# FlowEternal/multitask-hydranet

Hardware: AMD Instinct MI355X
Metric: images/sec (fwd+bwd) HydraNet @ default res, 1/2/4/8 MI355X; CPU-ref same run (higher is better)
Workload: dtype bf16

## Files before the change

### multitask_hydranet_amd/csrc/hn_gemm.hip

```cpp
#include "hn_common.h"
#include <climits>

#ifdef HN_TUNING
#define HN_DBG(p) ((p).dbg)
#else
#define HN_DBG(p) 0
#endif

struct XSrc {
    const bf16* x0;
    const bf16* x1;
    int mode;
    int H, W;
    int Hi, Wi;
    int C0, C1;
    int ld0, ld1;
    int up;
    long M;
    int clamp;
    int diag;
};

__device__ __forceinline__ int border_idx(int v, int L, int clamp) {
    if (clamp == 2) return (v < 0 || v >= L) ? -1 : v;
// ... 20 lines not shown
        iy = iy < 0 ? -iy : (iy >= s.Hi ? 2 * s.Hi - 2 - iy : iy);
        ix = ix < 0 ? -ix : (ix >= s.Wi ? 2 * s.Wi - 2 - ix : ix);
        if (c < s.C0) {
            const int hh = s.Hi >> s.up, ww = s.Wi >> s.up;
            return ld8(s.x0 + (((long)n * hh + (iy >> s.up)) * ww + (ix >> s.up)) * s.ld0 + c);
        }
        return ld8(s.x1 + (((long)n * s.Hi + iy) * s.Wi + ix) * s.ld1 + (c - s.C0));
    }
    const int iy = oy - ky, ix = ox - kx;
    if (iy < 0 || iy >= s.Hi || ix < 0 || ix >= s.Wi) return zero8();
    return ld8(s.x0 + (((long)n * s.Hi + iy) * s.Wi + ix) * s.ld0 + c);
}

__device__ __attribute__((aligned(16))) bf16 g_zero_piece[8];

__device__ __forceinline__ const bf16* x_piece_ptr(const XSrc& s, long m, int n, int oy, int ox, int tap, int c) {
    if (m >= s.M || c >= s.C0 + s.C1) return g_zero_piece;
    if (s.mode == 0) return s.x0 + m * s.ld0 + c;
    if (s.mode == 1) return s.x0 + (((long)n * s.Hi + 2 * oy) * s.Wi + 2 * ox) * s.ld0 + c;
    const int ky = (tap * 11) >> 5, kx = tap - 3 * ky;
    if (s.mode == 2) {
        int iy = oy + ky - 1, ix = ox + kx - 1;
        iy = iy < 0 ? -iy : (iy >= s.Hi ? 2 * s.Hi - 2 - iy : iy);
        ix = ix < 0 ? -ix : (ix >= s.Wi ? 2 * s.Wi - 2 - ix : ix);
        if (c < s.C0) {
            const int hh = s.Hi >> s.up, ww = s.Wi >> s.up;
            return s.x0 + (((long)n * hh + (iy >> s.up)) * ww + (ix >> s.up)) * s.ld0 + c;
        }
        return s.x1 + (((long)n * s.Hi + iy) * s.Wi + ix) * s.ld1 + (c - s.C0);
    }
    const int iy = oy - ky, ix = ox - kx;
    if (iy < 0 || iy >= s.Hi || ix < 0 || ix >= s.Wi) return g_zero_piece;
    return s.x0 + (((long)n * s.Hi + iy) * s.Wi + ix) * s.ld0 + c;
}

__device__ __forceinline__ long pixel_off(const XSrc& s, long m, int n, int oy, int ox, int tap, int which) {
    if (m >= s.M) return -1;
    if (s.mode == 0) return which ? -1 : m * s.ld0;
    if (s.mode == 1) return which ? -1 : (((long)n * s.Hi + 2 * oy) * s.Wi + 2 * ox) * s.ld0;
    const int ky = (tap * 11) >> 5, kx = tap - 3 * ky;
    if (s.mode == 2) {
        int iy = oy + ky - 1, ix = ox + kx - 1;
        iy = iy < 0 ? -iy : (iy >= s.Hi ? 2 * s.Hi - 2 - iy : iy);
        ix = ix < 0 ? -ix : (ix >= s.Wi ? 2 * s.Wi - 2 - ix : ix);
        if (which) return s.C1 ? (((long)n * s.Hi + iy) * s.Wi + ix) * s.ld1 : -1;
        const int hh = s.Hi >> s.up, ww = s.Wi >> s.up;
        return (((long)n * hh + (iy >> s.up)) * ww + (ix >> s.up)) * s.ld0;
    }
    const int iy = oy - ky, ix = ox - kx;
    if (which || iy < 0 || iy >= s.Hi || ix < 0 || ix >= s.Wi) return -1;
    return (((long)n * s.Hi + iy) * s.Wi + ix) * s.ld0;
}

__device__ __forceinline__ void glds16(const bf16* src, char* lds_wave_base) {
    __builtin_amdgcn_global_load_lds((const __attribute__((address_space(1))) void*)src,
                                     (__attribute__((address_space(3))) void*)lds_wave_base, 16, 0, 0);
}

__device__ __forceinline__ int swz(int row, int piece) { return row * 128 + ((piece ^ (row & 7)) << 4); }
__device__ __forceinline__ int pswz32(int row) { return (row >> 1) & 2; }

struct GemmNT {
    XSrc x;
    const bf16* w;
    int Nout, KP, taps;
    const float* bias;
    int act;
    void* out;
    int ldc;
    float* psum;
    float* psq;
    long rpi;
    long img_stride;
    int d2s;
    const float* xscale; const float* xshift; const float* xgate; long xhw; int xact;
    const bf16* addend; int ld_add;
    int phase_mode, phase_span;
    int add_s2;
    long* amax;
    int add_pre;
    long w_img_stride; unsigned w_rpi;
    const float* lcoef; int ln; long lrow[HN_MAX_LEVELS + 1];
    int lo_n; unsigned lo_hw[HN_MAX_LEVELS]; unsigned lo_pix[HN_MAX_LEVELS];
    int fold;
    bf16* fold_out2; int ld_fo2;
    bf16* ring;
    const bf16* fold_y; int ld_fy;
    int emode; const bf16* ez; int ld_ez; const float* ecoef;
    const bf16* ey; int ld_ey;
    int tile_major;
    int wpre;
    unsigned long long* dbg_buf;
    int dbg;
};

struct StatCoef { f32x4 sc, sh, mu, rs; };
__device__ __forceinline__ StatCoef stat_coef(const float* ecoef, int Nout, int emode, int co0, bool ev) {
    StatCoef c;
    c.sc = c.sh = c.mu = c.rs = (f32x4){0.f, 0.f, 0.f, 0.f};
    if (ev) {
        c.sc = *reinterpret_cast<const f32x4*>(ecoef + co0);
        c.sh = *reinterpret_cast<const f32x4*>(ecoef + Nout + co0);
        if (emode == 2) {
            c.mu = *reinterpret_cast<const f32x4*>(ecoef + 2 * Nout + co0);
            c.rs = *reinterpret_cast<const f32x4*>(ecoef + 3 * Nout + co0);
        }
    }
    return c;
}
__device__ __forceinline__ void stat_terms4(int emode, const f32x4 q, const f32x4 z, const StatCoef& cf, float& a0, float& a1, float& a2, float& a3,
                                            float& b0, float& b1, float& b2, float& b3) {
    float t1[4], t2[4];
#pragma unroll
    for (int r = 0; r < 4; ++r) {
        const float pre = cf.sc[r] * z[r] + cf.sh[r];
        const float b = bfround(pre > 0.f ? pre : 0.f);
        const float g = pre > 0.f ? q[r] : 0.f;
        t1[r] = emode == 0 ? q[r] : (emode == 1 ? q[r] * b : g);
        t2[r] = emode == 0 ? q[r] * q[r] : g * (z[r] - cf.mu[r]) * cf.rs[r];
    }
    a0 += t1[0]; a1 += t1[1]; a2 += t1[2]; a3 += t1[3];
    b0 += t2[0]; b1 += t2[1]; b2 += t2[2]; b3 += t2[3];
}

template <int BC, int BP, int WGC, int WGP, bool OUT_F32, int R, bool XF = false, int KG = 1, bool PLAIN = false, bool EPRE = false>
__global__ __launch_bounds__(256 * KG) void gemm_nt_kernel(const GemmNT p) {
    static_assert(!XF || R == 2, "the register-staged operand transform is written for the double buffer");
    static_assert(!PLAIN || !XF, "the plain-rows form has no operand transform");
    static_assert(KG == 1 || (!XF && R == 2), "the K-group form is written for the plain double buffer");
    constexpr int WC = BC / WGC, WP = BP / WGP, TC = WC / 16, TP = WP / 16;
    constexpr int XR = BP / 32, WR = (BC + 31) / 32;
    constexpr int STAGE = (BC + BP) * 128;
    extern __shared__ __attribute__((aligned(16))) char smem[];
    const int tid = threadIdx.x & 255, kg = __builtin_amdgcn_readfirstlane(threadIdx.x >> 8), lane = tid & 63, wave = __builtin_amdgcn_readfirstlane(tid >> 6);
    const int wc = wave / WGP, wp = wave % WGP;
    const int ncy = (p.Nout + BC - 1) / BC;
    const int lid = xcd_remap(blockIdx.x, gridDim.x);
    const int c_tile = lid % ncy, p_tile = lid / ncy;
    const int c_blk = c_tile * BC;
    const long p_blk = (long)p_tile * BP;
    const int r0 = tid >> 3, lp = (tid & 7) ^ (r0 & 7), half = lp >> 2, sub = (lp & 3) * 8;
    const int kc = p.KP >> 5, Q = p.taps * kc, S = (((Q + 1) >> 1) + KG - 1) / KG;
    const int Ktot = p.taps * p.KP;

    int xn[XR], xy[XR], xx[XR];
#pragma unroll
    for (int i = 0; i < XR; ++i) {
        if constexpr (PLAIN) { xn[i] = 0; xy[i] = 0; xx[i] = 0; }
        else decomp_row(p.x, p_blk + r0 + 32 * i, xn[i], xy[i], xx[i]);
    }

    int* ty0 = reinterpret_cast<int*>(smem + R * KG * STAGE);
    int* tx0 = ty0 + 3 * p.x.H;
    int* ty1 = tx0 + 3 * p.x.W;
    int* tx1 = ty1 + 3 * p.x.H;
    if (!PLAIN && p.x.mode >= 2) {
        for (int i = tid; i < 3 * p.x.H; i += 256) {
            const int k = i / p.x.H, o = i - k * p.x.H;
            if (p.x.mode == 2) {
                int v = o + k - 1;
                v = border_idx(v, p.x.Hi, p.x.clamp);
                ty0[i] = v >> p.x.up;
                if (p.x.C1) ty1[i] = v;
            } else {
                const int v = o - k;
                ty0[i] = (v < 0 || v >= p.x.Hi) ? -1 : v;
            }
// ... 427 lines not shown
#pragma unroll
        for (int k = 0; k < WGP; ++k) { t1 += red[(k * BC + tid) * 2]; t2 += red[(k * BC + tid) * 2 + 1]; }
        p.psum[(long)p_tile * p.Nout + c_blk + tid] = t1;
        if (p.psq) p.psq[(long)p_tile * p.Nout + c_blk + tid] = t2;
    }
    if (staged) {
        bf16* outp = reinterpret_cast<bf16*>(p.out);
        float e1[8], e2[8], emu[8], ers[8];
#pragma unroll
        for (int k = 0; k < 8; ++k) { e1[k] = 0.f; e2[k] = 0.f; emu[k] = 0.f; ers[k] = 0.f; }
        if (e3) {
            const int co = c_blk + (tid % NPC) * 8;
            if (co < p.Nout) {
#pragma unroll
                for (int k = 0; k < 8; ++k) { emu[k] = p.ecoef[2 * p.Nout + co + k]; ers[k] = p.ecoef[3 * p.Nout + co + k]; }
            }
        }
#pragma unroll
        for (int u = 0; u < NIT; ++u) {
            const int idx = tid + 256 * u;
            if (idx >= BP * NPC) break;
            const int row = idx / NPC, pc = idx % NPC;
            const long pix = p_blk + row;
            const int co = c_blk + pc * 8;
            if (pix < p.x.M && co < p.Nout) {
                bf16x8 v = *reinterpret_cast<const bf16x8*>(smem + row * (BC * 2) + (((pc ^ row) & (NPC - 1)) << 4));
                long orow = pix * p.ldc;
                if (p.rpi) {
                    const unsigned im = (unsigned)pix / (unsigned)p.rpi;
                    orow = (long)im * p.img_stride + (long)((unsigned)pix - im * (unsigned)p.rpi) * p.ldc;
                }
                if (p.addend && !p.add_pre) {
                    bool has = true;
                    bf16x8 a;
                    if (PRE) {
                        has = phas[u < PRE ? u : 0];
                        a = padd[u < PRE ? u : 0];
                    } else {
                        long arow = pix;
                        if (p.add_s2) {
                            const unsigned W = (unsigned)p.x.W, H = (unsigned)p.x.H;
                            const unsigned x = (unsigned)pix % W, t = (unsigned)pix / W;
                            const unsigned y = t % H, n = t / H;
                            has = !((x | y) & 1u);
                            arow = ((long)n * (H >> 1) + (y >> 1)) * (W >> 1) + (x >> 1);
                        }
                        a = has ? ld8(p.addend + arow * p.ld_add + co) : zero8();
                    }
                    if (has) {
#pragma unroll
                        for (int k = 0; k < 8; ++k) v[k] = f2bf(bf2f(v[k]) + bf2f(a[k]));
                    }
                }
                if (e3) {
                    const bf16x8 yv = PRE ? pey[u < PRE ? u : 0] : ld8(p.ey + pix * p.ld_ey + co);
                    const bf16x8 zv = PRE ? pzz[u < PRE ? u : 0] : ld8(p.ez + pix * p.ld_ez + co);
#pragma unroll
                    for (int k = 0; k < 8; ++k) {
                        const float g = bf2f(yv[k]) > 0.f ? bf2f(v[k]) : 0.f;
                        e1[k] += g;
                        e2[k] += g * (bf2f(zv[k]) - emu[k]) * ers[k];
                    }
                }
                *reinterpret_cast<bf16x8*>(outp + orow + co) = v;
            }
        }
        if (e3) {
            float* r3 = reinterpret_cast<float*>(smem + BP * BC * 2 + WGP * BC * 8);
            static_assert(BP * BC * 2 + WGP * BC * 8 + 256 * 16 * 4 <= R * KG * STAGE || BC < 64, "emode 3 scratch fits the operand ring");
#pragma unroll
            for (int k = 0; k < 8; ++k) { r3[tid * 16 + k] = e1[k]; r3[tid * 16 + 8 + k] = e2[k]; }
            __syncthreads();
            if (tid < BC && c_blk + tid < p.Nout) {
                const int pc = tid >> 3, k = tid & 7;
                float t1 = 0.f, t2 = 0.f;
                for (int j = 0; j < 256 / NPC; ++j) { t1 += r3[(j * NPC + pc) * 16 + k]; t2 += r3[(j * NPC + pc) * 16 + 8 + k]; }
                p.psum[(long)p_tile * p.Nout + c_blk + tid] = t1;
                p.psq[(long)p_tile * p.Nout + c_blk + tid] = t2;
            }
        }
    }
}

template <int BC, bool OUT_F32, bool PIPE, int XB = (PIPE ? 2 : 1)>
__global__ __launch_bounds__(512, 4) void conv3x3_direct_kernel(const GemmNT p) {
    constexpr int KC = PIPE ? 32 : 64;
    constexpr int NPP = KC / 8, PB = KC * 2;
    constexpr int XBUFS = XB, WBUFS = PIPE ? 4 : 2;
    constexpr int WCO = BC >= 64 ? 64 : BC;
    constexpr int WGC = BC / WCO, WGP = 8 / WGC, ROWS = 16 / WGP;
    constexpr int TC = WCO / 16, TP = ROWS;
    constexpr int PPIX = 18 * 18, XL = (PPIX * NPP + 511) / 512, WL = (BC * NPP + 511) / 512;
    constexpr bool PRE32 = PIPE && XB == 1;
    constexpr int XBYTES = PIPE ? XL * 512 * 16 : (PPIX * 128 + 1023) / 1024 * 1024, WBYTES = PRE32 ? BC * PB : (PIPE ? WL * 512 * 16 : BC * 128);
    extern __shared__ __attribute__((aligned(16))) char smem[];
    char* sXb = smem;
    char* sWb = smem + XBUFS * XBYTES;
    const int tid = threadIdx.x, lane = tid & 63, wave = __builtin_amdgcn_readfirstlane(tid >> 6);
    const int wc = wave / WGP, wp = wave % WGP;
    const XSrc& xs = p.x;
    const int ncy = (p.Nout + BC - 1) / BC;
    const int tx_n = (xs.W + 15) >> 4, ty_n = (xs.H + 15) >> 4;
    const int lid = xcd_remap(blockIdx.x, gridDim.x);
    unsigned long long* stampb = (HN_DBG(p) & 16) && (blockIdx.x & 63) == 0 && tid == 0
                                     ? reinterpret_cast<unsigned long long*>(p.dbg_buf) + (blockIdx.x >> 6) * 128 : nullptr;
    int stampi = 0;
    auto stamp = [&]() {
#ifdef HN_TUNING
        __builtin_amdgcn_sched_barrier(0);
        if (stampb && stampi < 128) stampb[stampi++] = __builtin_amdgcn_s_memtime();
        __builtin_amdgcn_sched_barrier(0);
#endif
    };
    stamp();
    const int npatch = gridDim.x / ncy;
    const int c_tile = p.tile_major ? lid / npatch : lid % ncy;
    int t = p.tile_major ? lid % npatch : lid / ncy;
    const int patch_id = t;
    const int tx = t % tx_n;
    t /= tx_n;
    const int ty = t % ty_n;
    const int n = t / ty_n;
    const int c_blk = c_tile * BC, oy0 = ty * 16, ox0 = tx * 16;
    const int org = xs.mode == 2 ? -1 : -2;
    const int Ctot = xs.C0 + xs.C1;
    const int NT = p.phase_mode ? 4 : 9;
    const int nchunk = xs.diag ? 1 : (p.KP + KC - 1) / KC, S = nchunk * NT;
    const int Ktot = 9 * p.KP;
    const int tile_phase = p.phase_mode == 1 ? c_blk / p.phase_span : 0;
    const int cpp = p.phase_mode == 2 ? p.phase_span / KC : 0;
    struct Cur { int chunk, ti, ph, cnt; };
    auto cur0 = [&]() { Cur c; c.chunk = 0; c.ti = 0; c.ph = tile_phase; c.cnt = 0; return c; };
    auto adv = [&](Cur& c) {
        if (++c.ti == NT) {
            c.ti = 0;
            ++c.chunk;
            if (p.phase_mode == 2 && ++c.cnt == cpp) { c.cnt = 0; ++c.ph; }
        }
    };
    auto tap_at = [&](const Cur& c) { return p.phase_mode ? ((c.ph >> 1) + (c.ti >> 1)) * 3 + (c.ph & 1) + (c.ti & 1) : c.ti; };
    const int xc0 = xs.diag ? c_blk : 0;
    float* sbias = reinterpret_cast<float*>(smem + XBUFS * XBYTES + ((!PIPE || PRE32) && p.wpre ? S : WBUFS) * WBYTES);
    if (tid < BC) sbias[tid] = (p.bias && c_blk + tid < p.Nout) ? p.bias[c_blk + tid] : 0.f;

    if (BC == 64 && !PIPE && xs.diag) {
#pragma unroll
        for (int i = 0; i < 2; ++i) {
            if (512 * i + 64 * wave < 9 * 64) {
                const int e = 512 * i + tid, tap = e >> 6, col = e & 63, co = c_blk + col;
                const bf16* src = co < p.Nout ? p.w + co * (9 * p.KP) + tap * 64 + (col >> 3) * 8 : g_zero_piece;
                glds16(src, smem + XBUFS * XBYTES + (512 * i + 64 * wave) * 16);
            }
        }
    }
    int* patch_src = reinterpret_cast<int*>(sbias + BC);
    if (tid < 36) {
        const bool isy = tid < 18;
        const int k = isy ? tid : tid - 18, L = isy ? xs.Hi : xs.Wi;
        int g = (isy ? oy0 : ox0) + org + k;
        if (xs.mode == 2) g = border_idx(g, L, xs.clamp);
        else g = (g >= 0 && g < L) ? g : -1;
        patch_src[tid] = g;
    }
    __syncthreads();
    const bool single = xs.C1 == 0 && (long)p.x.M < (1L << 27);
    int spack[XL];
#pragma unroll
    for (int i = 0; i < XL; ++i) {
        const int e = tid + 512 * i;
        const int pp = e / NPP;
        spack[i] = -1;
        if (pp < PPIX) {
            const int py = pp / 18, px = pp - py * 18;
            const int sub = PIPE ? ((e & 3) ^ pswz32(px)) : ((e & 7) ^ (px & 7));
            const int gy = patch_src[py], gx = patch_src[18 + px];
            if ((gy | gx) >= 0)
                spack[i] = single ? ((((n * (xs.Hi >> xs.up) + (gy >> xs.up)) * (xs.Wi >> xs.up) + (gx >> xs.up)) << 3) | sub)
                                  : ((gy << 16) | (sub << 13) | gx);
        }
    }
    auto issue_x = [&](int chunk) {
        if ((HN_DBG(p) & 4) && chunk >= XBUFS) return;
        const int k0 = chunk * KC;
        char* sX = sXb + (XBUFS == 2 ? (chunk & 1) : 0) * XBYTES;
#pragma unroll
        for (int i = 0; i < XL; ++i) {
            if (PIPE || 512 * i + 64 * wave < PPIX * 8) {
                const bf16* src = g_zero_piece;
                int pk = spack[i];
                asm volatile("" : "+v"(pk));
                if (single) {
                    const int c = xc0 + k0 + ((pk & 7) << 3);
                    if (c < Ctot && pk >= 0) src = xs.x0 + c + (long)(pk >> 3) * xs.ld0;
                } else {
                    const int c = xc0 + k0 + (((pk >> 13) & 7) << 3);
                    if (c < Ctot && pk >= 0) {
                        const int gy = pk >> 16, gx = pk & 0x1fff;
                        if (c < xs.C0) src = xs.x0 + c + (long)((n * (xs.Hi >> xs.up) + (gy >> xs.up)) * (xs.Wi >> xs.up) + (gx >> xs.up)) * xs.ld0;
                        else src = xs.x1 + (c - xs.C0) + (long)((n * xs.Hi + gy) * xs.Wi + gx) * xs.ld1;
                    }
                }
                glds16(src, sX + (512 * i + 64 * wave) * 16);
            }
        }
    };
    const bool early_x = ((!PIPE || PRE32) && p.wpre) || (BC == 64 && !PIPE && xs.diag);
    if (early_x) issue_x(0);
    const int wsub = PIPE ? (((tid & 3) ^ pswz32(tid >> 2)) << 3) : (((tid & 7) ^ ((tid >> 3) & 7)) << 3);
    int wrow[WL];
#pragma unroll
    for (int i = 0; i < WL; ++i) {
        const int r = tid / NPP + (512 / NPP) * i;
        const int co = c_blk + r;
        wrow[i] = (r < BC && co < p.Nout) ? co * Ktot + wsub : -1;
    }

    f32x4 acc[TC][TP];
#pragma unroll
    for (int i = 0; i < TC; ++i)
#pragma unroll
        for (int j = 0; j < TP; ++j) acc[i][j] = (f32x4){0.f, 0.f, 0.f, 0.f};

    const int aofs = PIPE ? (wc * WCO + (lane & 15)) * PB + (((lane >> 4) ^ pswz32(lane & 15)) << 4) : swz(wc * WCO + (lane & 15), lane >> 4);
    int bofs[3];
#pragma unroll
    for (int d = 0; d < 3; ++d) {
        const int pc = (lane & 15) + d;
        bofs[d] = (wp * ROWS * 18 + pc) * PB + (PIPE ? (((lane >> 4) ^ pswz32(pc)) << 4) : (((lane >> 4) ^ (pc & 7)) << 4));
    }

    const bool rows_live = oy0 + wp * ROWS < xs.H;
    auto compute = [&](const Cur& c, int slot) {
        if (!rows_live) return;
        const int tap = tap_at(c);
        const int ky = (tap * 11) >> 5, kx = tap - 3 * ky;
        const int dy = xs.mode == 2 ? ky : 2 - ky, dx = xs.mode == 2 ? kx : 2 - kx;
        const int wo = slot * WBYTES + aofs;
        const int xo = (XBUFS == 2 ? (c.chunk & 1) : 0) * XBYTES + dy * (18 * PB) + (dx == 0 ? bofs[0] : (dx == 1 ? bofs[1] : bofs[2]));
#pragma unroll
        for (int ks = 0; ks < KC / 32; ++ks) {
            bf16x8 a[TC], b[TP];
            const int wk = ks ? (wo ^ 64) : wo, xk = ks ? (xo ^ 64) : xo;
#pragma unroll
            for (int i = 0; i < TC; ++i) a[i] = (HN_DBG(p) & 8) ? zero8() : *reinterpret_cast<const bf16x8*>(sWb + wk + i * 16 * PB);
#pragma unroll
            for (int j = 0; j < TP; ++j) b[j] = (HN_DBG(p) & 8) ? zero8() : *reinterpret_cast<const bf16x8*>(sXb + xk + j * 18 * PB);
            if (HN_DBG(p) & 2) {
#pragma unroll
                for (int i = 0; i < (TC < TP ? TC : TP); ++i) asm volatile("" :: "v"(a[i]), "v"(b[i]));
                continue;
            }
#pragma unroll
            for (int i = 0; i < TC; ++i)
#pragma unroll
                for (int j = 0; j < TP; ++j)
                    acc[i][j] = __builtin_amdgcn_mfma_f32_16x16x32_bf16(a[i], b[j], acc[i][j], 0, 0, 0);
        }
    };
    auto issue_w = [&](const Cur& c, int slot, int seq) {
        if ((HN_DBG(p) & 4) && seq >= WBUFS) return;
        const int k0 = c.chunk * KC;
        const int koff = tap_at(c) * p.KP + k0;
        char* sW = sWb + slot * WBYTES;
#pragma unroll
        for (int i = 0; i < WL; ++i) {
            if ((PIPE && !PRE32) || wave * (64 / NPP) + (512 / NPP) * i < BC) {
                const bf16* src = (wrow[i] >= 0 && k0 + wsub < p.KP) ? p.w + wrow[i] + koff : g_zero_piece;
                glds16(src, sW + (512 * i + 64 * wave) * 16);
            }
        }
    };
    const int ox = ox0 + (lane & 15);
    const bool pre_add = !OUT_F32 && p.d2s && p.addend;
    constexpr int AQ = 2;
    bf16x4 addq[AQ][TP];
    auto load_add = [&](int i, bf16x4 (&dst)[TP]) {
        const int co0 = c_blk + wc * WCO + i * 16 + (lane >> 4) * 4;
        const int ph = co0 / p.d2s, oc = co0 - ph * p.d2s;
#pragma unroll
        for (int j = 0; j < TP; ++j) {
            const int oy = oy0 + wp * ROWS + j;
            const long opix = ((long)(n * 2 * xs.H + 2 * oy + (ph >> 1)) * (2 * xs.W) + 2 * ox + (ph & 1));
            dst[j] = (oy < xs.H && ox < xs.W && co0 < p.Nout) ? *reinterpret_cast<const bf16x4*>(p.addend + opix * p.ld_add + oc)
                                                              : (bf16x4){(bf16)0.f, (bf16)0.f, (bf16)0.f, (bf16)0.f};
        }
    };
    bool add_issued = false;
    stamp();
    if ((!PIPE || PRE32) && p.wpre) {
        Cur ci = cur0();
        for (int st = 0; st < S; ++st) { issue_w(ci, st, 0); adv(ci); }
        asm volatile("s_waitcnt vmcnt(0)" ::: "memory");
        __syncthreads();
        stamp();
        Cur cc = cur0();
        if constexpr (PRE32) {
            if (S == 9 && p.phase_mode == 0) {
#pragma unroll
                for (int st = 0; st < 9; ++st) { compute(cc, st); adv(cc); }
            } else {
                for (int st = 0; st < S; ++st) { compute(cc, st); adv(cc); }
            }
        } else {
            for (int st = 0; st < S; ++st) { compute(cc, st); adv(cc); }
        }
    } else if (BC == 64 && !PIPE && xs.diag) {
        asm volatile("s_waitcnt vmcnt(0)" ::: "memory");
        __syncthreads();
        const int kq = lane >> 4;
        for (int tap = 0; tap < (rows_live ? 9 : 0); ++tap) {
            const int ky = (tap * 11) >> 5, kx = tap - 3 * ky;
            const int dy = xs.mode == 2 ? ky : 2 - ky, dx = xs.mode == 2 ? kx : 2 - kx;
            const int pxk = ((lane & 15) + dx) & 7;
#pragma unroll
// ... 282 lines not shown
                    }
                }
            } else if (OUT_F32) {
                float* o = reinterpret_cast<float*>(p.out) + orow + co0;
                if (co0 + 3 < p.Nout && (reinterpret_cast<uintptr_t>(o) & 15) == 0) *reinterpret_cast<f32x4*>(o) = (f32x4){v[0], v[1], v[2], v[3]};
                else {
#pragma unroll
                    for (int r = 0; r < 4; ++r) if (co0 + r < p.Nout) o[r] = v[r];
                }
            } else {
                bf16* o = reinterpret_cast<bf16*>(p.out) + orow + co0;
                if (stage_d2s) {
                    bf16x4 tv = {f2bf(v[0]), f2bf(v[1]), f2bf(v[2]), f2bf(v[3])};
                    const int pl = (wp * ROWS + j) * 16 + (lane & 15), cl = wc * WCO + i * 16 + (lane >> 4) * 4;
                    *reinterpret_cast<bf16x4*>(stage + pl * (BC * 2) + ((((cl >> 3) ^ pl) & (BC / 8 - 1)) << 4) + (cl & 7) * 2) = tv;
                } else if (co0 + 3 < p.Nout && (reinterpret_cast<uintptr_t>(o) & 7) == 0) {
                    bf16x4 tv = {f2bf(v[0]), f2bf(v[1]), f2bf(v[2]), f2bf(v[3])};
                    *reinterpret_cast<bf16x4*>(o) = tv;
                } else {
#pragma unroll
                    for (int r = 0; r < 4; ++r) if (co0 + r < p.Nout) o[r] = f2bf(v[r]);
                }
            }
        }
    }
    if (p.amax && !stage_f32) return;
    if (stage_f32 && p.amax) {
        __syncthreads();
        const int rowf = 32 * p.d2s;
        for (int idx = tid; idx < 32 * 32; idx += 512) {
            const int Y = idx >> 5, X = idx & 31;
            const int gy = 2 * oy0 + Y, gx = 2 * ox0 + X;
            if (gy < 2 * xs.H && gx < 2 * xs.W) {
                const float* r = reinterpret_cast<const float*>(stage) + Y * rowf + X * p.d2s;
                float best = r[0];
                int arg = 0;
                for (int c = 1; c < p.d2s; ++c)
                    if (r[c] > best) { best = r[c]; arg = c; }
                p.amax[(long)(n * 2 * xs.H + gy) * (2 * xs.W) + gx] = arg;
            }
        }
    } else if (stage_f32) {
        __syncthreads();
        const int rowf = 32 * p.d2s, row4 = rowf >> 2;
        float* ob = reinterpret_cast<float*>(p.out);
        for (int idx = tid; idx < 32 * row4; idx += 512) {
            const int Y = idx / row4, q4 = idx - Y * row4;
            const int gy = 2 * oy0 + Y;
            const int valid = (2 * xs.W - 2 * ox0) * p.d2s;
            if (gy < 2 * xs.H && q4 * 4 < valid) {
                float* dst = ob + ((long)(n * 2 * xs.H + gy) * (2 * xs.W) + 2 * ox0) * p.d2s + q4 * 4;
                const f32x4 v = *reinterpret_cast<const f32x4*>(reinterpret_cast<const float*>(stage) + Y * rowf + q4 * 4);
                if (q4 * 4 + 4 <= valid) *reinterpret_cast<f32x4*>(dst) = v;
                else for (int k = 0; q4 * 4 + k < valid; ++k) dst[k] = v[k];
            }
        }
    }
    stamp();
    if (stage_d2s) {
        __syncthreads();
        constexpr int NPC = BC / 8;
        const int ph = p.d2s ? c_blk / p.d2s : 0, oc0 = p.d2s ? c_blk - ph * p.d2s : c_blk;
        bf16* outp = reinterpret_cast<bf16*>(p.out);
        if (p.fold) {
            constexpr int ITER = 256 * NPC / 512;
            const int H = xs.H - 2, W = xs.W - 2;
            const int pc = tid % NPC, c = c_blk + pc * 8;
            long dst[ITER];
            bf16x8 yv[ITER];
#pragma unroll
            for (int i = 0; i < ITER; ++i) {
                const int pl = (tid + 512 * i) / NPC;
                const int oy = oy0 + (pl >> 4), oxx = ox0 + (pl & 15);
                const int iy = oy - 1, ix = oxx - 1;
                dst[i] = LONG_MIN;
                yv[i] = zero8();
                if (oy < xs.H && oxx < xs.W && c < p.Nout) {
                    if ((unsigned)iy < (unsigned)H && (unsigned)ix < (unsigned)W) {
                        const long pix = (long)(n * H + iy) * W + ix;
                        const long cell = (long)(n * (H >> 1) + (iy >> 1)) * (W >> 1) + (ix >> 1);
                        const int pch = ((iy & 1) * 2 + (ix & 1)) * p.Nout + c;
                        dst[i] = p.fold == 2 ? cell * p.ldc + pch : pix * p.ldc + c;
                        if (p.fold_y) yv[i] = ld8(p.fold_y + pix * p.ld_fy + c);
                    } else {
                        const int r = oy == 0 ? oxx : (oy == H + 1 ? xs.W + oxx : (oxx == 0 ? 2 * xs.W + iy : 2 * xs.W + H + iy));
                        dst[i] = -(((long)n * (2 * xs.W + 2 * H) + r) * p.Nout + c) - 1;
                    }
                }
            }
#pragma unroll
            for (int i = 0; i < ITER; ++i) {
                if (dst[i] == LONG_MIN) continue;
                const int pl = (tid + 512 * i) / NPC;
                bf16x8 v = *reinterpret_cast<const bf16x8*>(stage + pl * (BC * 2) + (((pc ^ pl) & (NPC - 1)) << 4));
                if (dst[i] >= 0) {
                    if (p.fold_y) {
#pragma unroll
                        for (int k = 0; k < 8; ++k) { const float yy = bf2f(yv[i][k]), f = bf2f(v[k]); v[k] = f2bf(yy > 0.f ? f : f * (yy + 1.0f)); }
                    }
                    *reinterpret_cast<bf16x8*>(outp + dst[i]) = v;
                    if (p.fold == 3) {
                        const int iy = oy0 + (pl >> 4) - 1, ix = ox0 + (pl & 15) - 1;
                        const long cell = (long)(n * (H >> 1) + (iy >> 1)) * (W >> 1) + (ix >> 1);
                        *reinterpret_cast<bf16x8*>(p.fold_out2 + cell * p.ld_fo2 + ((iy & 1) * 2 + (ix & 1)) * p.Nout + c) = v;
                    }
                } else {
                    *reinterpret_cast<bf16x8*>(p.ring - dst[i] - 1) = v;
                }
            }
            return;
        }
#pragma unroll 2
        for (int idx = tid; idx < 256 * NPC; idx += 512) {
            const int pl = idx / NPC, pc = idx - pl * NPC;
            const int oy = oy0 + (pl >> 4), oxx = ox0 + (pl & 15);
            if (oy < xs.H && oxx < xs.W && c_blk + pc * 8 < p.Nout) {
                const long opix = p.d2s ? ((long)(n * 2 * xs.H + 2 * oy + (ph >> 1)) * (2 * xs.W) + 2 * oxx + (ph & 1))
                                        : ((long)(n * xs.H + oy) * xs.W + oxx);
                const bf16x8 v = *reinterpret_cast<const bf16x8*>(stage + pl * (BC * 2) + (((pc ^ pl) & (NPC - 1)) << 4));
                *reinterpret_cast<bf16x8*>(outp + opix * p.ldc + oc0 + pc * 8) = v;
            }
        }
        asm volatile("s_waitcnt vmcnt(0)" ::: "memory");
        stamp();
    }
}

struct SegOut { const bf16* x; int ldx, N, H, W; const bf16* w; int Nout, k; const float* bias; float* out; long* amax; int npatch, ppw; };
template <bool AMAX>
__global__ __launch_bounds__(512, 2) void seg_out_conv_kernel(const SegOut p) {
    extern __shared__ __attribute__((aligned(16))) char smem[];
    constexpr int PPIX = 18 * 18, XCH = (PPIX * 8 + 63) / 64, XBYTES = XCH * 1024;
    const int tid = threadIdx.x, lane = tid & 63, wave = __builtin_amdgcn_readfirstlane(tid >> 6);
    float* stf = reinterpret_cast<float*>(smem + 2 * XBYTES);
    const int k = p.k, rowf = 32 * k;
    const int tx_n = (p.W + 15) >> 4, ty_n = (p.H + 15) >> 4;
    const int bidx = xcd_remap(blockIdx.x, gridDim.x);
    const int t0 = bidx * p.ppw;
    int t1 = t0 + p.ppw;
    if (t1 > p.npatch) t1 = p.npatch;
    if (t0 >= t1) return;
    bf16x8 wf[2][9][2];
#pragma unroll
    for (int i = 0; i < 2; ++i) {
        const int co = i * 16 + (lane & 15);
#pragma unroll
        for (int tap = 0; tap < 9; ++tap)
#pragma unroll
            for (int ks = 0; ks < 2; ++ks)
                wf[i][tap][ks] = co < p.Nout ? *reinterpret_cast<const bf16x8*>(p.w + ((long)co * 9 + tap) * 64 + ks * 32 + (lane >> 4) * 8) : zero8();
    }
    float bs[2][4];
#pragma unroll
    for (int i = 0; i < 2; ++i)
#pragma unroll
        for (int r = 0; r < 4; ++r) {
            const int co = i * 16 + (lane >> 4) * 4 + r;
            bs[i][r] = (p.bias && co < p.Nout) ? p.bias[co] : 0.f;
        }
    int req[6];
#pragma unroll
    for (int i = 0; i < 6; ++i) {
        const int e = (wave + 8 * i) * 64 + lane, pp = e >> 3;
        const int py = pp / 18, px = pp - py * 18;
        req[i] = (wave + 8 * i < XCH && pp < PPIX) ? ((py << 16) | (px << 8) | ((e & 7) ^ (px & 7))) : -1;
    }
    auto issue = [&](int t, char* sX) {
// ... 1502 lines not shown
#else
extern const long g_hn_knob[20] = {2048, 256, 1024, 512, 8192, 262144, 0, 0, 1, 0, 0, 0, 256, 384, 0, 0, 0, 0, 0, 0};
#endif
static bool small_tile(long M, int Nout) { return !g_nt_force_bc && Nout > 64 && (M <= g_hn_knob[4] || (M <= g_hn_knob[5] && Nout <= 128)); }

extern "C" int hn_direct_stat_rows(int n_img, int H, int W) { return n_img * cdiv(H, 16) * cdiv(W, 16); }

extern "C" int hn_nt_stat_rows(long M, int Nout) {
    return small_tile(M, Nout) ? cdiv(M, 64) : cdiv(M, 128);
}
extern "C" int hn_nt_stat_tile(long M, int Nout) { return small_tile(M, Nout) ? 64 : 128; }

static bool aligned16(const void* q) { return (reinterpret_cast<uintptr_t>(q) & 15) == 0; }

static GemmNT nt_desc(const XSrc& x, const void* w, int Nout, int KP, int taps, const float* bias, int act, void* out, int ldc) {
    GemmNT p{};
    p.x = x;
    p.w = (const bf16*)w; p.Nout = Nout; p.KP = KP; p.taps = taps;
    p.bias = bias; p.act = act; p.out = out; p.ldc = ldc;
    return p;
}

static GemmNT nt_rows(const void* x0, int ld0, long M, int C0, const void* w, int Nout, int KP, const float* bias, int act, void* out, int ldc) {
    return nt_desc(make_xsrc(x0, nullptr, 0, 0, 0, C0, 0, ld0, 0, 0, M), w, Nout, KP, 1, bias, act, out, ldc);
}

static GemmNT nt_conv(const void* x0, const void* x1, int mode, int H, int W, int C0, int C1, int ld0, int ld1, int up, long M, const void* w,
                      int Nout, int KP, int taps, const float* bias, int act, void* out, int ldc, long rpi, long img_stride, float* psum,
                      float* psq) {
    GemmNT p = nt_desc(make_xsrc(x0, x1, mode, H, W, C0, C1, ld0, ld1, up, M), w, Nout, KP, taps, bias, act, out, ldc);
    p.rpi = rpi; p.psum = psum; p.psq = psq;
    if (img_stride < 0) p.d2s = (int)(-img_stride);
    else p.img_stride = img_stride;
    return p;
}

static void nt_addend(GemmNT& p, const void* addend, int ld_add, int add_mode) {
    p.addend = (const bf16*)addend;
    p.ld_add = ld_add < 0 ? -ld_add : ld_add;
    p.add_pre = ld_add < 0 ? 1 : 0;
    p.add_s2 = add_mode;
}

static int launch_direct(GemmNT& p, int n_img, bool out_f32, hipStream_t st) {
    const XSrc& x = p.x;
    const long npatch = (long)cdiv(x.W, 16) * cdiv(x.H, 16) * n_img;
    if (x.clamp == 1 && !x.diag && !out_f32 && p.d2s == 64 && p.phase_mode == 1 && p.phase_span == 64 && p.taps == 9 && p.KP == 64 && x.C0 == 64 &&
        x.C1 == 0 && p.Nout == 256 && !p.psum && !p.addend && (p.act == HN_ACT_ELU || p.act == HN_ACT_NONE) && (x.ld0 & 7) == 0 &&
        (p.ldc & 7) == 0 && p.ldc >= 64 && aligned16(p.out) && g_hn_knob[11] != 3 && npatch >= 1024) {
        SegPhase q;
        q.x = x.x0; q.ldx = x.ld0; q.N = n_img; q.H = x.H; q.W = x.W; q.w = p.w; q.bias = p.bias; q.out = (bf16*)p.out; q.ldc = p.ldc;
        q.act = p.act; q.npatch = (int)npatch;
        q.ppw = cdiv(npatch, 64);
        const int grid = 4 * cdiv(npatch, q.ppw);
        const size_t lds = 2 * (size_t)((18 * 18 * 8 + 63) / 64) * 1024 + 256 * 128;
        static std::atomic<unsigned long long> optin_sp{0};
        if (!lds_optin(optin_sp, {(const void*)seg_phase64_conv_kernel})) return HN_ERR_LAUNCH;
        hipLaunchKernelGGL(seg_phase64_conv_kernel, dim3(grid), dim3(512), lds, st, q);
        HN_LAUNCH_CHECK();
    }
    if (x.clamp == 1 && !x.diag && out_f32 && p.d2s && p.taps == 9 && p.KP == 64 && x.C0 == 64 && x.C1 == 0 && p.Nout == 4 * p.d2s &&
        p.Nout <= 32 && !p.psum && !p.addend && p.phase_mode == 0 && p.act == HN_ACT_NONE && (x.ld0 & 7) == 0 && ((32 * p.d2s) & 3) == 0 &&
        ((2 * x.W * p.d2s) & 3) == 0 && aligned16(p.out) && g_hn_knob[11] != 3 && npatch >= 1024) {
        SegOut q;
        q.x = x.x0; q.ldx = x.ld0; q.N = n_img; q.H = x.H; q.W = x.W; q.w = p.w; q.Nout = p.Nout; q.k = p.d2s; q.bias = p.bias;
        q.out = p.amax ? nullptr : (float*)p.out; q.amax = p.amax; q.npatch = (int)npatch;
        q.ppw = cdiv(npatch, 256);
        const int grid = cdiv(npatch, q.ppw);
        const size_t lds = 2 * (size_t)((18 * 18 * 8 + 63) / 64) * 1024 + (size_t)32 * 32 * p.d2s * 4;
        static std::atomic<unsigned long long> optin_so{0};
        if (!lds_optin(optin_so, {(const void*)seg_out_conv_kernel<true>, (const void*)seg_out_conv_kernel<false>})) return HN_ERR_LAUNCH;
        if (p.amax) hipLaunchKernelGGL(seg_out_conv_kernel<true>, dim3(grid), dim3(512), lds, st, q);
        else hipLaunchKernelGGL(seg_out_conv_kernel<false>, dim3(grid), dim3(512), lds, st, q);
        HN_LAUNCH_CHECK();
    }
    HN_CHECK_ARG(x.Wi < 8192 && x.Hi < 32768);
    int bc = x.diag ? 64 : (p.Nout <= 16 ? 16 : (p.Nout <= 32 ? 32 : (p.Nout <= 64 ? 64 : 128)));
    if (p.phase_mode == 1 && p.phase_span < bc) bc = 64;
    const bool staged_ok = (p.ldc & 7) == 0 && (p.Nout & 7) == 0 && aligned16(p.out) && (!p.d2s || ((p.d2s & 7) == 0 && p.Nout % bc == 0));
    if (bc >= 64 && !out_f32 && !staged_ok) {
        if (x.diag) return HN_ERR_UNSUPPORTED;
        bc = 32;
    }
    dim3 grid((unsigned)(cdiv(p.Nout, bc) * cdiv(x.W, 16) * cdiv(x.H, 16) * n_img));
    const int nsteps = p.phase_mode ? 4 : 9;
    p.wpre = (!x.diag && p.KP <= 64 && (size_t)nsteps * bc * 128 <= 32768 && g_hn_knob[11] != 2) ? 1 : 0;
    const bool narrow = bc == 64 && !out_f32 && !x.diag && !p.wpre && p.KP <= 32 && nsteps == 9 && g_hn_knob[18] == 0;
    if (narrow) p.wpre = 1;
#ifdef HN_TUNING
    const bool pipe = narrow || (g_direct_pipe && bc >= 64 && !out_f32 && !x.diag && !p.wpre && p.KP > 64);
#else
    const bool pipe = narrow;
#endif
    const size_t lds = narrow ? (size_t)(((18 * 18 * 4 + 511) / 512) * 512 * 16) + 9 * (size_t)(64 * 64)
                     : pipe ? (size_t)2 * (((18 * 18 * 4 + 511) / 512) * 512 * 16) + 4 * (size_t)(512 * 16)
                            : (size_t)((18 * 18 * 128 + 1023) / 1024 * 1024) + (p.wpre ? nsteps : 2) * (size_t)bc * 128;
    const size_t lds_bias = (size_t)bc * 4 + 36 * 4;
    static std::atomic<unsigned long long> optin{0};
    if (!lds_optin(optin, {(const void*)conv3x3_direct_kernel<16, true, false>, (const void*)conv3x3_direct_kernel<16, false, false>,
                           (const void*)conv3x3_direct_kernel<32, true, false>, (const void*)conv3x3_direct_kernel<32, false, false>,
                           (const void*)conv3x3_direct_kernel<64, true, false>, (const void*)conv3x3_direct_kernel<64, false, false>,
                           (const void*)conv3x3_direct_kernel<128, true, false>, (const void*)conv3x3_direct_kernel<128, false, false>}))
        return HN_ERR_LAUNCH;
    if (narrow) {
        hipLaunchKernelGGL((conv3x3_direct_kernel<64, false, true, 1>), grid, dim3(512), lds + lds_bias, st, p);
        HN_LAUNCH_CHECK();
    }
#ifdef HN_TUNING
    static std::atomic<unsigned long long> optin_pipe{0};
    if (pipe) {
        if (!lds_optin(optin_pipe, {(const void*)conv3x3_direct_kernel<64, false, true>, (const void*)conv3x3_direct_kernel<128, false, true>}))
            return HN_ERR_LAUNCH;
        if (bc == 64) hipLaunchKernelGGL((conv3x3_direct_kernel<64, false, true>), grid, dim3(512), lds + lds_bias, st, p);
        else hipLaunchKernelGGL((conv3x3_direct_kernel<128, false, true>), grid, dim3(512), lds + lds_bias, st, p);
        HN_LAUNCH_CHECK();
    }
#endif
#define DIRECT_CASE(BC_) \
    if (bc == BC_) { \
        if (out_f32) hipLaunchKernelGGL((conv3x3_direct_kernel<BC_, true, false>), grid, dim3(512), lds + lds_bias, st, p); \
        else hipLaunchKernelGGL((conv3x3_direct_kernel<BC_, false, false>), grid, dim3(512), lds + lds_bias, st, p); \
    }
    DIRECT_CASE(16) DIRECT_CASE(32) DIRECT_CASE(64) DIRECT_CASE(128)
#undef DIRECT_CASE
    HN_LAUNCH_CHECK();
}

static int run_gemm_nt(GemmNT& p, int n_img, bool out_f32, hipStream_t st) {
    const XSrc& x = p.x;
    const int Nout = p.Nout, KP = p.KP, taps = p.taps;
    const long M = x.M;
    HN_CHECK_ARG(x.x0 && p.w && p.out && M > 0 && Nout > 0 && KP > 0 && (KP & 31) == 0 && taps >= 1 && taps <= 9);
    HN_CHECK_ARG(!p.xscale || (p.xshift && x.mode <= 1 && !out_f32 && x.C1 == 0 && (!p.xgate || p.xhw > 0)));
    HN_CHECK_ARG(p.phase_mode == 0 || ((x.mode == 3 || x.clamp == 1) && p.phase_span >= 64 && p.phase_span % 64 == 0 && !p.psum && !p.rpi));
    HN_CHECK_ARG(!p.addend || p.add_pre || (!out_f32 && (Nout & 7) == 0 && (p.ldc & 7) == 0 && (p.ld_add & 7) == 0 && p.rpi == 0 && x.mode <= 1 &&
                                            aligned16(p.out) && aligned16(p.addend)));
    HN_CHECK_ARG(!p.addend || !p.add_pre || ((x.mode <= 1 || p.phase_mode == 1) && p.rpi == 0 && (p.ld_add & 3) == 0));
    HN_CHECK_ARG((x.C0 & 7) == 0 && (x.C1 & 7) == 0 && (x.ld0 & 7) == 0 && (x.C1 == 0 || (x.x1 && (x.ld1 & 7) == 0)));
    HN_CHECK_ARG(x.mode >= 0 && x.mode <= 3 && (!x.clamp || (x.up == 0 && x.C1 == 0)));
    HN_CHECK_ARG(x.diag ? (KP == 64 && Nout == x.C0 && !p.rpi) : x.C0 + x.C1 <= KP);
    HN_CHECK_ARG(x.mode == 0 || (long)n_img * x.H * x.W == M);
    HN_CHECK_ARG(x.mode < 2 ? taps == 1 : taps == 9);
    HN_CHECK_ARG(x.mode != 2 || x.clamp || (x.H >= 2 && x.W >= 2));
    HN_CHECK_ARG(p.add_s2 == 0 || (p.add_s2 == 1 && p.addend && !p.add_pre && p.ld_add > 0 && x.mode == 0 && !(x.H & 1) && !(x.W & 1) &&
                                   (long)n_img * x.H * x.W == M && M < (1L << 32)));
    HN_CHECK_ARG(!p.lcoef || (x.mode == 0 && taps == 1 && !p.psum && !p.xscale));
    HN_CHECK_ARG(!p.lo_n || (x.mode == 0 && taps == 1 && out_f32 && !p.psum && !p.xscale && p.rpi == 0 && !p.addend && M < (1L << 32)));
    HN_CHECK_ARG(p.w_rpi == 0 || (x.mode == 0 && taps == 1 && !p.xscale && p.w_rpi % 128 == 0 && M < (1L << 32)));
    HN_CHECK_ARG(p.emode != 3 || (x.mode == 0 && taps == 1 && p.psum && p.psq && !out_f32 && p.addend && !p.add_pre && p.ld_add > 0 && !p.add_s2 &&
                                   (Nout & 7) == 0 && (p.ldc & 7) == 0 && p.rpi == 0 && aligned16(p.out) && small_tile(M, Nout)));
    HN_CHECK_ARG(!p.d2s || (x.clamp == 1 && (out_f32 || p.phase_mode == 1) && p.rpi == 0 && !p.psum && Nout == 4 * p.d2s));
    p.tile_major = g_hn_knob[11] == 1 ? 1 : 0;
    p.dbg = (int)g_hn_knob[14];
    p.dbg_buf = reinterpret_cast<unsigned long long*>(g_hn_knob[15]);
    if (x.mode >= 2 && (!p.psum || x.diag) && !p.rpi) return launch_direct(p, n_img, out_f32, st);
    if (p.xscale) {
#ifdef HN_TUNING
        if (small_tile(M, Nout)) return launch_nt_xf<64, 64, 2, 2>(p, st);
        switch (pick_bc(Nout)) {
            case 16: return launch_nt_xf<16, 128, 1, 4>(p, st);
            case 32: return launch_nt_xf<32, 128, 1, 4>(p, st);
            case 64: return launch_nt_xf<64, 128, 2, 2>(p, st);
            default: return launch_nt_xf<128, 128, 2, 2>(p, st);
        }
#else
        return HN_ERR_UNSUPPORTED;
#endif
    }
    if (small_tile(M, Nout)) {
        if (x.mode <= 1 && taps == 1 && KP >= (g_hn_knob[6] > 1 ? g_hn_knob[6] : 512) && g_hn_knob[6] != 1 && !g_nt_force_r)
            return launch_nt_r<64, 64, 2, 2, 2, 2>(p, out_f32, st);
        return launch_nt<64, 64, 2, 2>(p, out_f32, st);
    }
    switch (pick_bc(Nout)) {
        case 16: return launch_nt<16, 128, 1, 4>(p, out_f32, st);
        case 32: return launch_nt<32, 128, 1, 4>(p, out_f32, st);
        case 64: return launch_nt<64, 128, 2, 2>(p, out_f32, st);
        default: return launch_nt<128, 128, 2, 2>(p, out_f32, st);
    }
}

extern "C" int hn_conv_gemm_nt(const void* x0, const void* x1, int mode, int n_img, int H, int W, int C0, int C1, int ld0, int ld1,
                               int up, long M, const void* w, int Nout, int KP, int taps, const float* bias, int act, void* out,
                               int out_f32, int ldc, long rpi, long img_stride, float* psum, float* psq, hipStream_t st) {
    GemmNT p = nt_conv(x0, x1, mode, H, W, C0, C1, ld0, ld1, up, M, w, Nout, KP, taps, bias, act, out, ldc, rpi, img_stride, psum, psq);
    return run_gemm_nt(p, n_img, out_f32, st);
}

extern "C" int hn_conv_gemm_nt_imgw(const void* x0, int ld0, long M, int C0, const void* w, long w_img_stride, long rows_per_image, int Nout,
                                    int KP, const float* bias, int act, void* out, int ldc, const void* addend, int ld_add, hipStream_t st) {
    HN_CHECK_ARG(rows_per_image > 0 && rows_per_image % 128 == 0 && M % rows_per_image == 0 && w_img_stride >= (long)Nout * KP);
    HN_CHECK_ARG(!addend || ld_add > 0);
    GemmNT p = nt_rows(x0, ld0, M, C0, w, Nout, KP, bias, act, out, ldc);
    p.w_img_stride = w_img_stride; p.w_rpi = (unsigned)rows_per_image;
    if (addend) { p.addend = (const bf16*)addend; p.ld_add = ld_add; p.add_pre = 1; }
    return run_gemm_nt(p, 0, false, st);
}

extern "C" int hn_conv_gemm_nt_lvl(const void* x0, int ld0, long M, int C0, const void* w, int Nout, int KP, const float* bias, int act,
                                   void* out, int ldc, const float* coef, int nlev, const long* rows, hipStream_t st) {
    HN_CHECK_ARG(coef && rows && nlev >= 1 && nlev <= HN_MAX_LEVELS);
    GemmNT p = nt_rows(x0, ld0, M, C0, w, Nout, KP, bias, act, out, ldc);
    p.lcoef = coef; p.ln = nlev;
    for (int l = 0; l < nlev; ++l) {
// ... 667 lines not shown
```

Measured before the change: 986.8.

## Split fold conv border ring into dedicated register-only workgroups

For folded 3x3 direct convolutions with a channel block of 64 or more, the grid gains extra leading workgroups. These compute the one-pixel output border ring in a separate LDS-free path: MFMA on direct global loads, with taps skipped per wave using a ballot mask. The tiled workgroups are then shifted one pixel inward and cover only the interior, so they no longer handle boundary cases. This is meant to cut wasted tile work and per-pixel border handling in the main kernel. The cost is an extra kernel instantiation and ring workgroups that reload weights from global memory with little reuse.

```diff
diff --git a/multitask_hydranet_amd/csrc/hn_gemm.hip b/multitask_hydranet_amd/csrc/hn_gemm.hip
--- a/multitask_hydranet_amd/csrc/hn_gemm.hip
+++ b/multitask_hydranet_amd/csrc/hn_gemm.hip
@@ -126,7 +126,7 @@
     long w_img_stride; unsigned w_rpi;
     const float* lcoef; int ln; long lrow[HN_MAX_LEVELS + 1];
     int lo_n; unsigned lo_hw[HN_MAX_LEVELS]; unsigned lo_pix[HN_MAX_LEVELS];
-    int fold;
+    int fold, ring_wg;
     bf16* fold_out2; int ld_fo2;
     bf16* ring;
     const bf16* fold_y; int ld_fy;
@@ -720,7 +720,93 @@
     }
 }
 
-template <int BC, bool OUT_F32, bool PIPE, int XB = (PIPE ? 2 : 1)>
+template <int BC, int KC>
+__device__ __forceinline__ void direct_ring_item(const GemmNT& p, int rb) {
+    constexpr int WCO = BC >= 64 ? 64 : BC, WGC = BC / WCO, WGP = 8 / WGC, TC = WCO / 16;
+    const XSrc& xs = p.x;
+    const int lane = threadIdx.x & 63, wave = __builtin_amdgcn_readfirstlane(threadIdx.x >> 6);
+    const int wc = wave / WGP, wp = wave % WGP;
+    const int ncy = (p.Nout + BC - 1) / BC;
+    const int c_tile = rb % ncy, item = rb / ncy;
+    const int H = xs.H - 2, W = xs.W - 2, R = 2 * xs.W + 2 * H;
+    const long nring = xs.M / ((long)xs.H * xs.W) * R;
+    const long wave0 = (long)item * (16 * WGP) + wp * 16;
+    if (wave0 >= nring) return;
+    const long rp = wave0 + (lane & 15);
+    const bool live = rp < nring;
+    const int n = live ? (int)(rp / R) : 0, r = live ? (int)(rp - (long)n * R) : 0;
+    int y, x;
+    if (r < xs.W) { y = 0; x = r; }
+    else if (r < 2 * xs.W) { y = H + 1; x = r - xs.W; }
+    else if (r < 2 * xs.W + H) { y = r - 2 * xs.W + 1; x = 0; }
+    else { y = r - 2 * xs.W - H + 1; x = W + 1; }
+    unsigned tmask = 0;
+#pragma unroll
+    for (int tap = 0; tap < 9; ++tap) {
+        const int ky = (tap * 11) >> 5, kx = tap - 3 * ky;
+        const bool v = live && (unsigned)(y - ky) < (unsigned)xs.Hi && (unsigned)(x - kx) < (unsigned)xs.Wi;
+        if (__ballot(v)) tmask |= 1u << tap;
+    }
+    tmask = __builtin_amdgcn_readfirstlane(tmask);
+    const int Ctot = xs.C0, Ktot = 9 * p.KP, NT = p.phase_mode ? 4 : 9;
+    const int nchunk = (p.KP + KC - 1) / KC, cpp = p.phase_mode == 2 ? p.phase_span / KC : 1;
+    const int kq = (lane >> 4) * 8;
+    const int c_blk = c_tile * BC + wc * WCO;
+    const bf16* wrow[TC];
+#pragma unroll
+    for (int i = 0; i < TC; ++i) {
+        const int co = c_blk + i * 16 + (lane & 15);
+        wrow[i] = co < p.Nout ? p.w + (long)co * Ktot + kq : nullptr;
+    }
+    f32x4 acc[TC];
+#pragma unroll
+    for (int i = 0; i < TC; ++i) acc[i] = (f32x4){0.f, 0.f, 0.f, 0.f};
+    struct Step { int chunk, ti, ks; };
+    auto tap_of = [&](const Step& s) {
+        const int ph = p.phase_mode == 2 ? s.chunk / cpp : 0;
+        return p.phase_mode ? ((ph >> 1) + (s.ti >> 1)) * 3 + (ph & 1) + (s.ti & 1) : s.ti;
+    };
+    auto ok = [&](const Step& s) { return s.chunk * KC + s.ks * 32 < p.KP && ((tmask >> tap_of(s)) & 1); };
+    auto next = [&](Step& s) {
+        do {
+            if (++s.ks == KC / 32) { s.ks = 0; if (++s.ti == NT) { s.ti = 0; ++s.chunk; } }
+        } while (s.chunk < nchunk && !ok(s));
+    };
+    auto load = [&](const Step& s, bf16x8 (&a)[TC], bf16x8& b) {
+        const int tap = tap_of(s), k = s.chunk * KC + s.ks * 32;
+#pragma unroll
+        for (int i = 0; i < TC; ++i) a[i] = wrow[i] ? ld8(wrow[i] + tap * p.KP + k) : zero8();
+        const int ky = (tap * 11) >> 5, kx = tap - 3 * ky, iy = y - ky, ix = x - kx, c = k + kq;
+        const bool v = live && (unsigned)iy < (unsigned)xs.Hi && (unsigned)ix < (unsigned)xs.Wi && c < Ctot;
+        b = v ? ld8(xs.x0 + (((long)n * xs.Hi + iy) * xs.Wi + ix) * xs.ld0 + c) : zero8();
+    };
+    Step s = {0, 0, 0};
+    if (!ok(s)) next(s);
+    bf16x8 a0[TC], b0, a1[TC], b1;
+    if (s.chunk < nchunk) load(s, a0, b0);
+    while (s.chunk < nchunk) {
+        Step s1 = s;
+        next(s1);
+        if (s1.chunk < nchunk) load(s1, a1, b1);
+#pragma unroll
+        for (int i = 0; i < TC; ++i) acc[i] = __builtin_amdgcn_mfma_f32_16x16x32_bf16(a0[i], b0, acc[i], 0, 0, 0);
+        s = s1;
+#pragma unroll
+        for (int i = 0; i < TC; ++i) a0[i] = a1[i];
+        b0 = b1;
+    }
+    if (!live) return;
+#pragma unroll
+    for (int i = 0; i < TC; ++i) {
+        const int co0 = c_blk + i * 16 + (lane >> 4) * 4;
+        if (co0 < p.Nout) {
+            const f32x4 v = acc[i] + (f32x4){0.f, 0.f, 0.f, 0.f};
+            *reinterpret_cast<bf16x4*>(p.ring + rp * p.Nout + co0) = (bf16x4){f2bf(v[0]), f2bf(v[1]), f2bf(v[2]), f2bf(v[3])};
+        }
+    }
+}
+
+template <int BC, bool OUT_F32, bool PIPE, int XB = (PIPE ? 2 : 1), bool RING = false>
 __global__ __launch_bounds__(512, 4) void conv3x3_direct_kernel(const GemmNT p) {
     constexpr int KC = PIPE ? 32 : 64;
     constexpr int NPP = KC / 8, PB = KC * 2;
@@ -738,8 +824,14 @@
     const int wc = wave / WGP, wp = wave % WGP;
     const XSrc& xs = p.x;
     const int ncy = (p.Nout + BC - 1) / BC;
-    const int tx_n = (xs.W + 15) >> 4, ty_n = (xs.H + 15) >> 4;
-    const int lid = xcd_remap(blockIdx.x, gridDim.x);
+    const int ring_wg = RING ? p.ring_wg : 0, tiled = RING ? 1 : 0;
+    if (RING && (int)blockIdx.x < ring_wg) {
+        direct_ring_item<BC, KC>(p, blockIdx.x);
+        return;
+    }
+    const int tx_n = (xs.W - 2 * tiled + 15) >> 4, ty_n = (xs.H - 2 * tiled + 15) >> 4;
+    const int nwg = gridDim.x - ring_wg;
+    const int lid = xcd_remap(blockIdx.x - ring_wg, nwg);
     unsigned long long* stampb = (HN_DBG(p) & 16) && (blockIdx.x & 63) == 0 && tid == 0
                                      ? reinterpret_cast<unsigned long long*>(p.dbg_buf) + (blockIdx.x >> 6) * 128 : nullptr;
     int stampi = 0;
@@ -751,7 +843,7 @@
 #endif
     };
     stamp();
-    const int npatch = gridDim.x / ncy;
+    const int npatch = nwg / ncy;
     const int c_tile = p.tile_major ? lid / npatch : lid % ncy;
     int t = p.tile_major ? lid % npatch : lid / ncy;
     const int patch_id = t;
@@ -759,7 +851,7 @@
     t /= tx_n;
     const int ty = t % ty_n;
     const int n = t / ty_n;
-    const int c_blk = c_tile * BC, oy0 = ty * 16, ox0 = tx * 16;
+    const int c_blk = c_tile * BC, oy0 = ty * 16 + tiled, ox0 = tx * 16 + tiled;
     const int org = xs.mode == 2 ? -1 : -2;
     const int Ctot = xs.C0 + xs.C1;
     const int NT = p.phase_mode ? 4 : 9;
@@ -867,7 +959,7 @@
         bofs[d] = (wp * ROWS * 18 + pc) * PB + (PIPE ? (((lane >> 4) ^ pswz32(pc)) << 4) : (((lane >> 4) ^ (pc & 7)) << 4));
     }
 
-    const bool rows_live = oy0 + wp * ROWS < xs.H;
+    const bool rows_live = oy0 + wp * ROWS < xs.H - tiled;
     auto compute = [&](const Cur& c, int slot) {
         if (!rows_live) return;
         const int tap = tap_at(c);
@@ -1316,7 +1408,7 @@
                         const int pch = ((iy & 1) * 2 + (ix & 1)) * p.Nout + c;
                         dst[i] = p.fold == 2 ? cell * p.ldc + pch : pix * p.ldc + c;
                         if (p.fold_y) yv[i] = ld8(p.fold_y + pix * p.ld_fy + c);
-                    } else {
+                    } else if (!tiled) {
                         const int r = oy == 0 ? oxx : (oy == H + 1 ? xs.W + oxx : (oxx == 0 ? 2 * xs.W + iy : 2 * xs.W + H + iy));
                         dst[i] = -(((long)n * (2 * xs.W + 2 * H) + r) * p.Nout + c) - 1;
                     }
@@ -2985,7 +3077,16 @@
         if (x.diag) return HN_ERR_UNSUPPORTED;
         bc = 32;
     }
-    dim3 grid((unsigned)(cdiv(p.Nout, bc) * cdiv(x.W, 16) * cdiv(x.H, 16) * n_img));
+    const int ncy = cdiv(p.Nout, bc);
+    long tiles = (long)ncy * cdiv(x.W, 16) * cdiv(x.H, 16) * n_img;
+    p.ring_wg = 0;
+    if (p.fold && bc >= 64 && !out_f32 && g_hn_knob[19] == 0) {
+        const long nring = (long)n_img * (2 * x.W + 2 * (x.H - 2));
+        const int per_item = 16 * (bc >= 128 ? 4 : 8);
+        p.ring_wg = (int)((long)ncy * cdiv(nring, per_item) + 7) & ~7;
+        tiles = (long)ncy * cdiv(x.W - 2, 16) * cdiv(x.H - 2, 16) * n_img;
+    }
+    dim3 grid((unsigned)(tiles + p.ring_wg));
     const int nsteps = p.phase_mode ? 4 : 9;
     p.wpre = (!x.diag && p.KP <= 64 && (size_t)nsteps * bc * 128 <= 32768 && g_hn_knob[11] != 2) ? 1 : 0;
     const bool narrow = bc == 64 && !out_f32 && !x.diag && !p.wpre && p.KP <= 32 && nsteps == 9 && g_hn_knob[18] == 0;
@@ -3003,10 +3104,12 @@
     if (!lds_optin(optin, {(const void*)conv3x3_direct_kernel<16, true, false>, (const void*)conv3x3_direct_kernel<16, false, false>,
                            (const void*)conv3x3_direct_kernel<32, true, false>, (const void*)conv3x3_direct_kernel<32, false, false>,
                            (const void*)conv3x3_direct_kernel<64, true, false>, (const void*)conv3x3_direct_kernel<64, false, false>,
-                           (const void*)conv3x3_direct_kernel<128, true, false>, (const void*)conv3x3_direct_kernel<128, false, false>}))
+                           (const void*)conv3x3_direct_kernel<128, true, false>, (const void*)conv3x3_direct_kernel<128, false, false>,
+                           (const void*)conv3x3_direct_kernel<64, false, false, 1, true>, (const void*)conv3x3_direct_kernel<128, false, false, 1, true>}))
         return HN_ERR_LAUNCH;
     if (narrow) {
-        hipLaunchKernelGGL((conv3x3_direct_kernel<64, false, true, 1>), grid, dim3(512), lds + lds_bias, st, p);
+        if (p.ring_wg) hipLaunchKernelGGL((conv3x3_direct_kernel<64, false, true, 1, true>), grid, dim3(512), lds + lds_bias, st, p);
+        else hipLaunchKernelGGL((conv3x3_direct_kernel<64, false, true, 1>), grid, dim3(512), lds + lds_bias, st, p);
         HN_LAUNCH_CHECK();
     }
 #ifdef HN_TUNING
@@ -3023,6 +3126,11 @@
     if (bc == BC_) { \
         if (out_f32) hipLaunchKernelGGL((conv3x3_direct_kernel<BC_, true, false>), grid, dim3(512), lds + lds_bias, st, p); \
         else hipLaunchKernelGGL((conv3x3_direct_kernel<BC_, false, false>), grid, dim3(512), lds + lds_bias, st, p); \
+    }
+    if (p.ring_wg) {
+        if (bc == 64) hipLaunchKernelGGL((conv3x3_direct_kernel<64, false, false, 1, true>), grid, dim3(512), lds + lds_bias, st, p);
+        else hipLaunchKernelGGL((conv3x3_direct_kernel<128, false, false, 1, true>), grid, dim3(512), lds + lds_bias, st, p);
+        HN_LAUNCH_CHECK();
     }
     DIRECT_CASE(16) DIRECT_CASE(32) DIRECT_CASE(64) DIRECT_CASE(128)
 #undef DIRECT_CASE
```

Measured after the change: 990.0, median of 6. Within noise of the previous version (+0.3%).
